# EricBAndrews/Fast-Needleman-Wunsch

Measured on AMD Instinct MI355X. Metric: GCUPS (DP cell updates/s) on NxN NW fill, bit-exact score, higher is better.
Workload: dtype int32; 1 GPU; nw_fill_262144x262144; n1=262144, n2=262144, table_bytes=274880004100, layout=row-major int32, pitch 262208, waves=auto, parallelism=single GPU, kernel=panels

## Files before the change

fast-needleman-wunsch_amd/csrc/nw_sw.hip:

```cpp
#include <hip/hip_runtime.h>
#include <stdint.h>

#include <algorithm>

#include "nw_internal.h"

namespace nw {

__global__ __launch_bounds__(256) void nw_sw_best(const int32_t *__restrict__ smax, int32_t nstrips,
                                                  int32_t *__restrict__ best, uint64_t *__restrict__ key) {
    __shared__ int32_t red[256];
    int32_t m = 0;
    for (int32_t p = threadIdx.x; p < nstrips; p += 256) m = max(m, smax[p]);
    red[threadIdx.x] = m;
    __syncthreads();
    for (int s = 128; s > 0; s >>= 1) {
        if ((int)threadIdx.x < s) red[threadIdx.x] = max(red[threadIdx.x], red[threadIdx.x + s]);
        __syncthreads();
    }
    if (threadIdx.x == 0) {
        best[0] = red[0];
        *key = ~0ull;
    }
}

constexpr int kLocRows = 64;
constexpr int kLocMaxGrid = 4096;
__global__ __launch_bounds__(256) void nw_sw_locate(const int32_t *__restrict__ table, int64_t pitch,
                                                    int64_t n1, int64_t n2, int64_t col0, int32_t strip_cols,
                                                    const int32_t *__restrict__ smax, int32_t nstrips,
                                                    const int32_t *__restrict__ best,
                                                    uint64_t *__restrict__ key) {
    const int32_t b = *best;
    if (b <= 0) return;
    __shared__ unsigned long long kmin;
    if (threadIdx.x == 0) kmin = ~0ull;
    __syncthreads();
    const int64_t nblk = (n2 + kLocRows) / kLocRows;
    for (int64_t y = blockIdx.x; y < nblk; y += gridDim.x) {
        const int64_t r0 = y * kLocRows;
        const int nr = (int)min((int64_t)kLocRows, n2 + 1 - r0);
        for (int32_t p = 0; p < nstrips; ++p) {
            if (smax[p] != b) continue;
            for (int32_t x = threadIdx.x; x < strip_cols; x += 256) {
                const int64_t c = col0 + (int64_t)p * strip_cols + x;
                if (c > n1) break;
                const int32_t *col = table + r0 * pitch + c;
                int first = kLocRows;
#pragma unroll 16
                for (int rr = kLocRows - 1; rr >= 0; --rr) {
                    const int32_t v = rr < nr ? col[rr * pitch] : 0;
                    first = v == b ? rr : first;
                }
                if (first < kLocRows)
                    atomicMin(&kmin, ((unsigned long long)(r0 + first) << 32) | (unsigned long long)c);
            }
        }
    }
    __syncthreads();
    if (threadIdx.x == 0 && kmin != ~0ull) atomicMin((unsigned long long *)key, kmin);
}

int launch_sw_locate(const int32_t *table, int64_t pitch, int64_t n1, int64_t n2, int64_t col0,
                     int32_t strip_cols, const int32_t *smax, int32_t nstrips, uint64_t *key, int32_t *best,
                     void *stream) {
    hipStream_t s = (hipStream_t)stream;
    hipLaunchKernelGGL(nw_sw_best, dim3(1), dim3(256), 0, s, smax, nstrips, best, key);
    const int64_t grid = std::min<int64_t>((n2 + kLocRows) / kLocRows, kLocMaxGrid);
    hipLaunchKernelGGL(nw_sw_locate, dim3((unsigned)grid), dim3(256), 0, s, table, pitch, n1, n2, col0, strip_cols,
                       smax, nstrips, best, key);
    return (int)hipGetLastError();
}

__global__ __launch_bounds__(64) void nw_sw_fixup(int32_t *__restrict__ t, int64_t pitch,
                                                  const uint8_t *__restrict__ s1, const uint8_t *__restrict__ s2,
                                                  int32_t match, int32_t mismatch, int32_t gap, int64_t i0,
                                                  int64_t i1, int64_t j0, int64_t j1, int64_t col0, int32_t width,
                                                  int32_t *__restrict__ smax) {
    if (threadIdx.x != 0) return;
    for (int64_t i = i0; i <= i1; ++i) {
        int32_t left = t[i * pitch + j0 - 1];
        for (int64_t j = j0; j <= j1; ++j) {
            const int32_t d = t[(i - 1) * pitch + j - 1], u = t[(i - 1) * pitch + j];
            const int32_t sc = s1[j - 1] == s2[i - 1] ? match : mismatch;
            const int32_t v = max(max(0, d + sc), max(u + gap, left + gap));
            t[i * pitch + j] = v;
            left = v;
            atomicMax(smax + (j - col0) / width, v);
        }
    }
}

int64_t sw_half_corner(int32_t match, int32_t mismatch, int64_t n1, int64_t n2, int64_t *k) {
    const int64_t m = std::max(match, mismatch);
    if (m <= 0) {
        *k = INT64_MAX;
        return 0;
    }
    *k = (65536 + m - 1) / m;
    return std::max<int64_t>(0, n2 - *k + 1) * std::max<int64_t>(0, n1 - *k + 1);
}

int launch_sw_fixup(int32_t *table, int64_t pitch, int64_t n1, int64_t n2, const uint8_t *s1, const uint8_t *s2,
                    int32_t match, int32_t mismatch, int32_t gap, int64_t col0, int32_t strip_cols, int32_t *smax,
                    void *stream) {
    int64_t k = 0;
    if (sw_half_corner(match, mismatch, n1, n2, &k) == 0) return (int)hipSuccess;
    hipLaunchKernelGGL(nw_sw_fixup, dim3(1), dim3(64), 0, (hipStream_t)stream, table, pitch, s1, s2, match,
                       mismatch, gap, k, n2, k, n1, col0, strip_cols, smax);
    return (int)hipGetLastError();
}

constexpr int kTbR = 64;
constexpr int kTbBMax = 256;
constexpr int kTbWMax = 2 * kTbBMax + 1;
constexpr int kTbThreads = 512;
constexpr int kChain = 32;
enum : uint8_t { kCStop = 0, kCDiag = 1, kCUp = 2, kCLeft = 3, kCBad = 4 };
enum : uint32_t { kXCont = 0, kXStop = 1, kXOut = 2, kXBad = 3 };
__device__ __forceinline__ uint32_t xrec(uint32_t kind, uint32_t cnt, uint32_t r, uint32_t x) {
    return kind | (cnt << 2) | (r << 12) | (x << 19);
}

enum : int { kTbLocal = 0, kTbGlobal = 1, kTbBlock = 2 };

__host__ __device__ __forceinline__ int64_t tb_shift(int64_t k, int64_t is, int64_t js, int32_t B, int32_t aim,
                                                     int64_t row0 = 0) {
    if (!aim) return 0;
    const int64_t gi = is + row0;
    const int64_t num = js - gi, lim = B / 2;
    const int64_t mag = num < 0 ? -num : num;
    if (kTbR * mag > lim * gi) return (num < 0 ? -k : k) * lim;
    return k * kTbR * num / gi;
}

template <typename F>
__device__ __forceinline__ uint32_t tb_walk(const uint8_t *cd, int W, int x, F &&emit) {
    int r = kTbR - 1;
    uint32_t cnt = 0;
    for (;;) {
        const uint8_t c = cd[r * W + x];
        if (c == kCStop) return xrec(kXStop, cnt, r, x);
        if (c == kCBad) return xrec(kXBad, cnt, r, x);
        const int nx = c == kCUp ? x + 1 : c == kCLeft ? x - 1 : x;
        if (nx < 0 || nx >= W) return xrec(kXOut, cnt, r, x);
        emit(c == kCDiag ? 0u : c == kCUp ? 1u : 2u);
        ++cnt;
        if (c != kCLeft && r == 0) return xrec(kXCont, cnt, 0, nx);
        r = c == kCLeft ? r : r - 1;
        x = nx;
    }
}

template <int KIND>
__global__ __launch_bounds__(kTbThreads) void nw_tb_windows(const int32_t *__restrict__ table, int64_t pitch,
                                                            int64_t n1, const uint8_t *__restrict__ s1,
                                                            const uint8_t *__restrict__ s2, int32_t match,
                                                            int32_t mismatch, int32_t gap, int64_t is, int64_t js,
                                                            int32_t B, int32_t aim, int64_t row0,
                                                            uint8_t *__restrict__ codes,
                                                            uint32_t *__restrict__ exits) {
    __shared__ uint8_t cd[kTbR * kTbWMax];
    const int W = 2 * B + 1;
    const int k = blockIdx.x;
    const int64_t i0 = is - (int64_t)(k + 1) * kTbR + 1;
    const int64_t dj = js - is + i0 - B - tb_shift(k, is, js, B, aim, row0);
    const int ncell = kTbR * W;
    uint8_t *gcd = codes + (int64_t)k * ncell;
#pragma unroll 4
    for (int e = threadIdx.x; e < ncell; e += kTbThreads) {
        const int r = e / W, x = e - r * W;
        const int64_t i = i0 + r, j = dj + r + x;
        const bool in = i >= 1 && j >= 1 && j <= n1;
        const int64_t ic = in ? i : 1, jc = in ? j : 1;
        const int32_t *row = table + ic * pitch;
        const int32_t t = row[jc], td = row[jc - 1 - pitch], tu = row[jc - pitch], tl = row[jc - 1];
        const int32_t sc = s1[jc - 1] == s2[ic - 1] ? match : mismatch;
        const uint8_t mv = t == td + sc ? kCDiag : t == tu + gap ? kCUp : t == tl + gap ? kCLeft : kCBad;
        uint8_t c;
        if (KIND == kTbLocal) {
            c = in && t > 0 ? mv : kCStop;
        } else if (KIND == kTbBlock) {
            c = in ? mv
                   : i == 0 && j >= 0 && j <= n1 ? kCStop
                   : j == 0 && i > 0 ? kCUp
                                     : kCBad;
        } else {
            c = in ? mv
                   : i == 0 && j == 0 ? kCStop
                   : i == 0 && j > 0 && j <= n1 ? kCLeft
                   : j == 0 && i > 0 ? kCUp
                                     : kCBad;
        }
        cd[e] = c;
        gcd[e] = c;
    }
    __syncthreads();
    for (int x = threadIdx.x; x < W; x += kTbThreads) exits[(int64_t)k * W + x] = tb_walk(cd, W, x, [](uint32_t) {});
}

__global__ __launch_bounds__(1024) void nw_tb_chain(const uint32_t *__restrict__ exits, int32_t nwin, int32_t B,
                                                    int32_t aim, int64_t is, int64_t js, int64_t row0,
                                                    int64_t ops_cap, int64_t *__restrict__ wentry,
                                                    int64_t *__restrict__ ctl) {
    __shared__ uint32_t ex[kChain * kTbWMax];
    __shared__ int64_t st[3];
    const int W = 2 * B + 1;
    const int tid = threadIdx.x;
    if (tid == 0) {
        st[0] = B;
        st[1] = ctl[0];
        st[2] = 0;
    }
    for (int k0 = 0; k0 < nwin; k0 += kChain) {
        const int nk = min(kChain, nwin - k0);
        for (int e = tid; e < nk * W; e += 1024) ex[e] = exits[(int64_t)k0 * W + e];
        __syncthreads();
        if (tid == 0) {
            int x = (int)st[0];
            int64_t off = st[1];
            for (int kk = 0; kk < nk; ++kk) {
                const int k = k0 + kk;
                wentry[2 * k] = x;
                wentry[2 * k + 1] = off;
                const uint32_t rec = ex[kk * W + x];
                const uint32_t kind = rec & 3u, cnt = (rec >> 2) & 1023u, r = (rec >> 12) & 127u, xx = rec >> 19;
                off += cnt;
                const int64_t ck = tb_shift(k, is, js, B, aim, row0);
                x = (int)xx;
                if (kind == kXCont && k + 1 < nwin) {
                    x += (int)(tb_shift(k + 1, is, js, B, aim, row0) - ck);
                    if (x >= 0 && x < W) continue;
                }
                const int64_t i0 = is - (int64_t)(k + 1) * kTbR + 1, dj = js - is + i0 - B - ck;
                ctl[1] = off > ops_cap ? 4 : (int64_t)kind;
                ctl[2] = kind == kXCont ? i0 - 1 : i0 + r;
                ctl[3] = kind == kXCont ? dj - 1 + xx : dj + r + xx;
                ctl[4] = k + 1;
                ctl[0] = off;
                st[2] = 1;
                break;
            }
            st[0] = x;
            st[1] = off;
        }
        __syncthreads();
        if (st[2]) break;
    }
}

__global__ __launch_bounds__(256) void nw_tb_emit(const uint8_t *__restrict__ codes, int32_t B,
                                                  const int64_t *__restrict__ wentry, const int64_t *__restrict__ ctl,
                                                  uint8_t *__restrict__ ops) {
    __shared__ uint32_t cdw[kTbR * kTbWMax / 4 + 1];
    __shared__ uint8_t ob[2 * kTbR + kTbWMax + 8];
    __shared__ int32_t nop;
    const int k = blockIdx.x;
    if (k >= ctl[4] || ctl[1] == 4) return;
    const int W = 2 * B + 1, ncell = kTbR * W;
    const uint32_t *g = (const uint32_t *)(codes + (int64_t)k * ncell);
    for (int e = threadIdx.x; e < ncell / 4; e += 256) cdw[e] = g[e];
    __syncthreads();
    if (threadIdx.x == 0) {
        int q = 0;
        tb_walk((const uint8_t *)cdw, W, (int)wentry[2 * k], [&](uint32_t op) { ob[q++] = (uint8_t)op; });
        nop = q;
    }
    __syncthreads();
    const int64_t off = wentry[2 * k + 1];
    for (int m = threadIdx.x; m < nop; m += 256) ops[off + m] = ob[m];
}

size_t sw_tb_scratch_bytes(int32_t maxwin, int32_t band) {
    const size_t W = 2 * (size_t)band + 1;
    return 64 + (size_t)maxwin * (16 + 4 * W + kTbR * W);
}

static int32_t tb_steep_cap(int64_t is, int64_t js, int32_t B, int64_t row0) {
    const int64_t gi = is + row0;
    const int64_t num = js - gi, mag = num < 0 ? -num : num, lim = B / 2;
    const int64_t drift = (kTbR * mag - lim * gi) / gi;
    return drift <= 0 ? INT32_MAX : (int32_t)std::min<int64_t>(B / drift + 2, INT32_MAX);
}

template <int KIND>
static int run_traceback(const int32_t *table, int64_t pitch, int64_t n1, const uint8_t *s1, const uint8_t *s2,
                         int32_t match, int32_t mismatch, int32_t gap, int64_t end_i, int64_t end_j, uint8_t *ops,
                         int64_t ops_cap, void *scratch, int32_t maxwin, int32_t band, int32_t aim, int64_t *info,
                         void *stream, int64_t row0 = 0) {
    hipStream_t s = (hipStream_t)stream;
    for (int q = 0; q < 10; ++q) info[q] = 0;
    if (band < 1 || band > kTbBMax || maxwin < 1) return (int)hipErrorInvalidValue;
    const int W = 2 * band + 1;
    int64_t *ctl = (int64_t *)scratch;
    int64_t *wentry = ctl + 8;
    uint32_t *exits = (uint32_t *)(wentry + 2 * (size_t)maxwin);
    uint8_t *codes = (uint8_t *)(exits + (size_t)maxwin * W);
    hipError_t e = hipMemsetAsync(ctl, 0, 64, s);
    if (e != hipSuccess) return (int)e;
    int64_t ci = end_i, cj = end_j, h[8] = {0, 0, 0, 0, 0, 0, 0, 0};
    for (;;) {
        if (ci <= 0 || cj <= 0) {
            info[1] = ci;
            info[2] = cj;
            break;
        }
        int32_t nwin = (int32_t)std::min<int64_t>((ci + kTbR) / kTbR, maxwin);
        if (aim) nwin = std::min(nwin, tb_steep_cap(ci, cj, band, row0));
        hipLaunchKernelGGL(nw_tb_windows<KIND>, dim3((unsigned)nwin), dim3(kTbThreads), 0, s, table, pitch, n1, s1,
                           s2, match, mismatch, gap, ci, cj, band, aim, row0, codes, exits);
        hipLaunchKernelGGL(nw_tb_chain, dim3(1), dim3(1024), 0, s, exits, nwin, band, aim, ci, cj, row0, ops_cap,
                           wentry, ctl);
        hipLaunchKernelGGL(nw_tb_emit, dim3((unsigned)nwin), dim3(256), 0, s, codes, band, wentry, ctl, ops);
        if ((e = hipGetLastError()) != hipSuccess) return (int)e;
        if ((e = hipMemcpyAsync(h, ctl, sizeof h, hipMemcpyDeviceToHost, s)) != hipSuccess) return (int)e;
        if ((e = hipStreamSynchronize(s)) != hipSuccess) return (int)e;
        info[4] += 1;
        info[5] += nwin;
        info[0] = h[0];
        if (h[1] == kXStop) {
            info[1] = h[2];
            info[2] = h[3];
            break;
        }
        if (h[1] == kXBad || h[1] == 4) {
            info[3] = h[1] == 4 ? 1 : 2;
            info[1] = h[2];
            info[2] = h[3];
            break;
        }
        ci = h[2];
        cj = h[3];
    }
    if ((KIND == kTbGlobal || (KIND == kTbBlock && info[1] > 0)) && info[3] == 0 && (info[1] > 0 || info[2] > 0)) {
        const int64_t tail = info[1] > 0 ? info[1] : info[2];
        if (info[1] < 0 || info[2] < 0 || (info[1] > 0 && info[2] > 0)) {
            info[3] = 2;
        } else if (info[0] + tail > ops_cap) {
            info[3] = 1;
        } else {
            if ((e = hipMemsetAsync(ops + info[0], info[1] > 0 ? 1 : 2, (size_t)tail, s)) != hipSuccess)
                return (int)e;
            info[0] += tail;
            info[6] = tail;
            info[1] = info[2] = 0;
        }
    }
    return (int)hipSuccess;
}

int run_sw_traceback(const int32_t *table, int64_t pitch, int64_t n1, const uint8_t *s1, const uint8_t *s2,
                     int32_t match, int32_t mismatch, int32_t gap, int64_t end_i, int64_t end_j, uint8_t *ops,
                     int64_t ops_cap, void *scratch, int32_t maxwin, int32_t band, int64_t *info, void *stream) {
    return run_traceback<kTbLocal>(table, pitch, n1, s1, s2, match, mismatch, gap, end_i, end_j, ops, ops_cap, scratch,
                                   maxwin, band, 0, info, stream);
}

int run_nw_traceback(const int32_t *table, int64_t pitch, int64_t n1, int64_t n2, const uint8_t *s1,
                     const uint8_t *s2, int32_t match, int32_t mismatch, int32_t gap, uint8_t *ops, int64_t ops_cap,
                     void *scratch, int32_t maxwin, int32_t band, int32_t aim, int64_t *info, void *stream) {
    return run_traceback<kTbGlobal>(table, pitch, n1, s1, s2, match, mismatch, gap, n2, n1, ops, ops_cap, scratch,
                                    maxwin, band, aim, info, stream);
}

int run_nw_traceback_block(const int32_t *table, int64_t pitch, int64_t n1, int64_t rows, int64_t row0,
                           const uint8_t *s1, const uint8_t *s2, int32_t match, int32_t mismatch, int32_t gap,
                           uint8_t *ops, int64_t ops_cap, void *scratch, int32_t maxwin, int32_t band, int32_t aim,
                           int64_t *info, void *stream) {
    return run_traceback<kTbBlock>(table, pitch, n1, s1, s2, match, mismatch, gap, rows, n1, ops, ops_cap, scratch,
                                   maxwin, band, aim, info, stream, row0);
}

int64_t tb_shift_host(int64_t k, int64_t is, int64_t js, int32_t B, int32_t aim, int64_t row0) {
    return tb_shift(k, is, js, B, aim, row0);
}

}
```

fast-needleman-wunsch_amd/csrc/nw_traceback.cpp:

```cpp
#include <algorithm>
#include <cstring>

#include "nw_host_int.h"

using namespace nwh;

namespace {

int tb_workspace(nw_ctx *c, size_t ops, int64_t rows, int32_t band, int32_t *maxwin) {
    int st;
    if ((st = grow((void **)&c->ops, &c->ops_cap, ops)) != NW_OK) return st;
    *maxwin = (int32_t)std::min<int64_t>(*maxwin, rows / 64 + 1);
    return grow((void **)&c->tbscratch, &c->tbscratch_cap, nw::sw_tb_scratch_bytes(*maxwin, band));
}

int tb_elapsed(nw_ctx *c, hipStream_t s, float *ms) {
    NW_HIP_TRY(hipEventRecord(c->ev1, s));
    NW_HIP_TRY(hipStreamSynchronize(s));
    NW_HIP_TRY(hipEventElapsedTime(ms, c->ev0, c->ev1));
    return NW_OK;
}

void set_alignment(nw_alignment *out, int64_t end_i, int64_t end_j, const int64_t *info, float ms, int status) {
    out->end_i = end_i;
    out->end_j = end_j;
    out->n_ops = info[0];
    out->begin_i = info[1];
    out->begin_j = info[2];
    out->traceback_ms = ms;
    out->status = status;
}

}

extern "C" {

int nw_sw_traceback(nw_ctx *c, const int8_t *d_s1, int64_t n1, const int8_t *d_s2, int64_t n2,
                    const nw_params *p, const int32_t *d_t, int64_t pitch, int64_t end_i, int64_t end_j,
                    uint8_t *host_ops, int64_t ops_cap, nw_alignment *out) {
    if (!c || !d_t || !p || !out || n1 < 0 || n2 < 0 || end_i < 0 || end_j < 0 || end_i > n2 || end_j > n1)
        return NW_ERR_ARG;
    if ((end_j > 0 && !d_s1) || (end_i > 0 && !d_s2) || (ops_cap > 0 && !host_ops) || ops_cap < 0)
        return NW_ERR_ARG;
    if (!valid_params(p) || p->mode != NW_MODE_SW) return NW_ERR_ARG;
    NW_HIP_TRY(hipSetDevice(c->device));
    NW_HIP_TRY(hipDeviceSynchronize());
    const int32_t band = std::max(1, std::min(256, env_int("NW_TB_BAND", nw::kTbBandDefault)));
    int32_t maxwin = std::max(1, env_int("NW_TB_MAXWIN", nw::kTbMaxWinDefault));
    int st;
    const size_t need = (size_t)std::max<int64_t>(end_i + end_j + 1, 1);
    if ((st = tb_workspace(c, need, end_i, band, &maxwin)) != NW_OK) return st;
    NW_HIP_TRY(hipEventRecord(c->ev0, nullptr));
    int64_t info[10];
    const int he = nw::run_sw_traceback(d_t, pitch, n1, (const uint8_t *)d_s1, (const uint8_t *)d_s2, p->match,
                                        p->mismatch, p->gap, end_i, end_j, c->ops, (int64_t)need, c->tbscratch,
                                        maxwin, band, info, nullptr);
    if (he != hipSuccess) {
        std::fprintf(stderr, "libnwhip: SW traceback failed: %s\n", hipGetErrorString((hipError_t)he));
        return NW_ERR_HIP;
    }
    float ms = 0.f;
    if ((st = tb_elapsed(c, nullptr, &ms)) != NW_OK) return st;
    if (env_set("NW_TB_DEBUG"))
        std::fprintf(stderr, "nw_sw_traceback: %lld moves, %lld rounds, %lld windows (band %d)\n", (long long)info[0],
                     (long long)info[4], (long long)info[5], band);
    std::memset(out, 0, sizeof *out);
    set_alignment(out, end_i, end_j, info, ms, info[3] == 0 ? NW_OK : NW_ERR_HIP);
    NW_HIP_TRY(hipMemcpy(&out->score, d_t + end_i * pitch + end_j, 4, hipMemcpyDeviceToHost));
    if (info[3] != 0) return out->status;
    if (info[0] > ops_cap) return NW_ERR_ARG;
    if (info[0] > 0) {
        NW_HIP_TRY(hipMemcpy(host_ops, c->ops, (size_t)info[0], hipMemcpyDeviceToHost));
        std::reverse(host_ops, host_ops + info[0]);
    }
    return NW_OK;
}

int nw_traceback(nw_ctx *c, const int8_t *d_s1, int64_t n1, const int8_t *d_s2, int64_t n2, const nw_params *p,
                 const int32_t *d_t, int64_t pitch, const nw_tb_opts *o, void *stream, uint8_t *host_ops,
                 int64_t ops_cap, nw_alignment *out, nw_tb_stats *stats) {
    int32_t band = 0, maxwin = 0, aim = 0;
    int st = tb_args(n1, n2, p, o, host_ops, ops_cap, out, &band, &maxwin, &aim);
    if (st != NW_OK) return st;
    if (!c || !d_t || pitch < n1 + 1 || (n1 > 0 && !d_s1) || (n2 > 0 && !d_s2)) return NW_ERR_ARG;
    hipStream_t s = (hipStream_t)stream;
    NW_HIP_TRY(hipSetDevice(c->device));
    if ((st = tb_workspace(c, (size_t)std::max<int64_t>(n1 + n2, 1), n2, band, &maxwin)) != NW_OK) return st;
    NW_HIP_TRY(hipEventRecord(c->ev0, s));
    int64_t info[10];
    const int he = nw::run_nw_traceback(d_t, pitch, n1, n2, (const uint8_t *)d_s1, (const uint8_t *)d_s2, p->match,
                                        p->mismatch, p->gap, c->ops, n1 + n2, c->tbscratch, maxwin, band, aim, info,
                                        stream);
    if (he != hipSuccess) {
        std::fprintf(stderr, "libnwhip: traceback failed: %s\n", hipGetErrorString((hipError_t)he));
        return NW_ERR_HIP;
    }
    std::memset(out, 0, sizeof *out);
    out->end_i = n2;
    out->end_j = n1;
    if (stats) {
        stats->rounds = (int32_t)info[4];
        stats->windows = (int32_t)info[5];
        stats->band = band;
        stats->max_windows = maxwin;
        stats->tail_ops = info[6];
    }
    const bool ok = info[3] == 0;
    NW_HIP_TRY(hipMemcpyAsync(&out->score, d_t + n2 * pitch + n1, 4, hipMemcpyDeviceToHost, s));
    if (ok && info[0] > 0) NW_HIP_TRY(hipMemcpyAsync(host_ops, c->ops, (size_t)info[0], hipMemcpyDeviceToHost, s));
    float ms = 0.f;
    if ((st = tb_elapsed(c, s, &ms)) != NW_OK) return st;
    if (!ok) {
        out->traceback_ms = ms;
        out->status = NW_ERR_TABLE;
        return NW_ERR_TABLE;
    }
    set_alignment(out, n2, n1, info, ms, NW_OK);
    std::reverse(host_ops, host_ops + info[0]);
    return NW_OK;
}

int nw_traceback_block(nw_ctx *c, const int8_t *d_s1, int64_t n1, const int8_t *d_s2_block, int64_t rows,
                       int64_t row0, const nw_params *p, const int32_t *d_t, int64_t pitch, const nw_tb_opts *o,
                       void *stream, uint8_t *host_ops, int64_t ops_cap, nw_alignment *out, nw_tb_stats *stats) {
    int32_t band = 0, maxwin = 0, aim = 0;
    int st = tb_args(n1, rows, p, o, host_ops, ops_cap, out, &band, &maxwin, &aim);
    if (st != NW_OK) return st;
    if (row0 < 0 || row0 + rows >= INT32_MAX) return NW_ERR_ARG;
    if (!c || !d_t || pitch < n1 + 1 || (n1 > 0 && !d_s1) || (rows > 0 && !d_s2_block)) return NW_ERR_ARG;
    if (row0 == 0) {
        st = nw_traceback(c, d_s1, n1, d_s2_block, rows, p, d_t, pitch, o, stream, host_ops, ops_cap, out, stats);
        return st;
    }
    hipStream_t s = (hipStream_t)stream;
    NW_HIP_TRY(hipSetDevice(c->device));
    if ((st = tb_workspace(c, (size_t)std::max<int64_t>(n1 + rows, 1), rows, band, &maxwin)) != NW_OK) return st;
    NW_HIP_TRY(hipEventRecord(c->ev0, s));
    int64_t info[10];
    const int he = nw::run_nw_traceback_block(d_t, pitch, n1, rows, row0, (const uint8_t *)d_s1,
                                              (const uint8_t *)d_s2_block, p->match, p->mismatch, p->gap, c->ops,
                                              n1 + rows, c->tbscratch, maxwin, band, aim, info, stream);
    if (he != hipSuccess) {
        std::fprintf(stderr, "libnwhip: traceback failed: %s\n", hipGetErrorString((hipError_t)he));
        return NW_ERR_HIP;
    }
    std::memset(out, 0, sizeof *out);
    if (stats) {
        stats->rounds = (int32_t)info[4];
        stats->windows = (int32_t)info[5];
        stats->band = band;
        stats->max_windows = maxwin;
        stats->tail_ops = info[6];
    }
    const bool ok = info[3] == 0;
    NW_HIP_TRY(hipMemcpyAsync(&out->score, d_t + rows * pitch + n1, 4, hipMemcpyDeviceToHost, s));
    if (ok && info[0] > 0) NW_HIP_TRY(hipMemcpyAsync(host_ops, c->ops, (size_t)info[0], hipMemcpyDeviceToHost, s));
    float ms = 0.f;
    if ((st = tb_elapsed(c, s, &ms)) != NW_OK) return st;
    if (!ok) {
        out->end_i = row0 + rows;
        out->end_j = n1;
        out->traceback_ms = ms;
        out->status = NW_ERR_TABLE;
        return NW_ERR_TABLE;
    }
    set_alignment(out, row0 + rows, n1, info, ms, NW_OK);
    out->begin_i = row0 + info[1];
    std::reverse(host_ops, host_ops + info[0]);
    return NW_OK;
}

int64_t nw_debug_tb_shift(int64_t k, int64_t is, int64_t js, int32_t band, int32_t aim, int64_t row0) {
    return nw::tb_shift_host(k, is, js, band, aim, row0);
}

}
```

Baseline: 1522 GCUPS.

## Batch traceback rounds on device and stage window table reads through LDS rows

Traceback now keeps its loop state on the device: a begin kernel seeds the control block, and the window and chain kernels read their position from it and exit early once finished. The host enqueues growing batches of rounds between synchronisations instead of one sync per round. The window kernel loads table rows into a shared-memory ring with prefetch instead of doing four scattered global loads per cell, and the score is returned through the control block. None of this touches the fill kernel that the GCUPS metric measures, and speculative batches launch idle kernels.

```diff
diff --git a/fast-needleman-wunsch_amd/csrc/nw_sw.hip b/fast-needleman-wunsch_amd/csrc/nw_sw.hip
--- a/fast-needleman-wunsch_amd/csrc/nw_sw.hip
+++ b/fast-needleman-wunsch_amd/csrc/nw_sw.hip
@@ -2,6 +2,7 @@
 #include <stdint.h>
 
 #include <algorithm>
+#include <cstdlib>
 
 #include "nw_internal.h"
 
@@ -114,7 +115,7 @@
 constexpr int kTbR = 64;
 constexpr int kTbBMax = 256;
 constexpr int kTbWMax = 2 * kTbBMax + 1;
-constexpr int kTbThreads = 512;
+constexpr int kTbThreads = 576;
 constexpr int kChain = 32;
 enum : uint8_t { kCStop = 0, kCDiag = 1, kCUp = 2, kCLeft = 3, kCBad = 4 };
 enum : uint32_t { kXCont = 0, kXStop = 1, kXOut = 2, kXBad = 3 };
@@ -137,80 +138,188 @@
 template <typename F>
 __device__ __forceinline__ uint32_t tb_walk(const uint8_t *cd, int W, int x, F &&emit) {
     int r = kTbR - 1;
+    int at = r * W + x;
     uint32_t cnt = 0;
     for (;;) {
-        const uint8_t c = cd[r * W + x];
+        const uint32_t c = cd[at];
         if (c == kCStop) return xrec(kXStop, cnt, r, x);
         if (c == kCBad) return xrec(kXBad, cnt, r, x);
-        const int nx = c == kCUp ? x + 1 : c == kCLeft ? x - 1 : x;
-        if (nx < 0 || nx >= W) return xrec(kXOut, cnt, r, x);
-        emit(c == kCDiag ? 0u : c == kCUp ? 1u : 2u);
+        const int dx = (c == kCUp) - (c == kCLeft), nx = x + dx;
+        if ((unsigned)nx >= (unsigned)W) return xrec(kXOut, cnt, r, x);
+        emit(c - kCDiag);
         ++cnt;
-        if (c != kCLeft && r == 0) return xrec(kXCont, cnt, 0, nx);
-        r = c == kCLeft ? r : r - 1;
+        if (c != kCLeft) {
+            if (r == 0) return xrec(kXCont, cnt, 0, nx);
+            --r;
+            at -= W;
+        }
+        at += dx;
         x = nx;
     }
 }
+static_assert(kCDiag == 1 && kCUp == 2 && kCLeft == 3, "tb_walk emits code - 1");
+
+__host__ __device__ __forceinline__ bool tb_running(int64_t state) { return state == kXCont || state == kXOut; }
+
+__host__ __device__ __forceinline__ int32_t tb_steep_cap(int64_t is, int64_t js, int32_t B, int64_t row0) {
+    const int64_t gi = is + row0;
+    const int64_t num = js - gi, mag = num < 0 ? -num : num, lim = B / 2;
+    const int64_t drift = (kTbR * mag - lim * gi) / gi;
+    if (drift <= 0) return INT32_MAX;
+    const int64_t cap = B / drift + 2;
+    return cap < INT32_MAX ? (int32_t)cap : INT32_MAX;
+}
+
+__host__ __device__ __forceinline__ int32_t tb_nwin(int64_t is, int64_t js, int32_t B, int32_t aim, int64_t row0,
+                                                    int32_t maxwin) {
+    int64_t n = (is + kTbR) / kTbR;
+    n = n < maxwin ? n : maxwin;
+    if (aim) {
+        const int32_t cap = tb_steep_cap(is, js, B, row0);
+        n = n < cap ? n : cap;
+    }
+    return (int32_t)n;
+}
+
+__global__ void nw_tb_begin(const int32_t *__restrict__ table, int64_t pitch, int64_t ci, int64_t cj,
+                            int64_t *__restrict__ ctl) {
+    if (threadIdx.x != 0) return;
+    ctl[0] = 0;
+    ctl[1] = ci <= 0 || cj <= 0 ? kXStop : kXCont;
+    ctl[2] = ci;
+    ctl[3] = cj;
+    ctl[4] = ctl[5] = ctl[6] = 0;
+    ctl[7] = table[ci * pitch + cj];
+}
+
+constexpr int kTbCh = 8;
+constexpr int kTbRingW = kTbWMax + 3;
+constexpr int kTbLd = (kTbWMax + 2 + 63) / 64;
+constexpr int kTbAhead = 2;
+static_assert(kTbR % kTbCh == 0 && (kTbR * kTbWMax) % 4 == 0 && kTbThreads >= 64 * kTbCh && kTbThreads >= kTbWMax,
+              "window chunks");
 
 template <int KIND>
 __global__ __launch_bounds__(kTbThreads) void nw_tb_windows(const int32_t *__restrict__ table, int64_t pitch,
                                                             int64_t n1, const uint8_t *__restrict__ s1,
                                                             const uint8_t *__restrict__ s2, int32_t match,
-                                                            int32_t mismatch, int32_t gap, int64_t is, int64_t js,
-                                                            int32_t B, int32_t aim, int64_t row0,
+                                                            int32_t mismatch, int32_t gap, int32_t B, int32_t aim,
+                                                            int64_t row0, int32_t maxwin,
+                                                            const int64_t *__restrict__ ctl,
                                                             uint8_t *__restrict__ codes,
                                                             uint32_t *__restrict__ exits) {
-    __shared__ uint8_t cd[kTbR * kTbWMax];
+    __shared__ uint32_t cdw[kTbR * kTbWMax / 4];
+    __shared__ int32_t ring[(kTbCh + 1) * kTbRingW];
+    __shared__ uint8_t s1c[kTbR + kTbWMax];
+    if (!tb_running(ctl[1])) return;
+    const int64_t is = ctl[2], js = ctl[3];
+    const int k = blockIdx.x;
+    if (k >= tb_nwin(is, js, B, aim, row0, maxwin)) return;
+    uint8_t *cd = (uint8_t *)cdw;
     const int W = 2 * B + 1;
-    const int k = blockIdx.x;
     const int64_t i0 = is - (int64_t)(k + 1) * kTbR + 1;
     const int64_t dj = js - is + i0 - B - tb_shift(k, is, js, B, aim, row0);
     const int ncell = kTbR * W;
-    uint8_t *gcd = codes + (int64_t)k * ncell;
-#pragma unroll 4
-    for (int e = threadIdx.x; e < ncell; e += kTbThreads) {
-        const int r = e / W, x = e - r * W;
-        const int64_t i = i0 + r, j = dj + r + x;
-        const bool in = i >= 1 && j >= 1 && j <= n1;
-        const int64_t ic = in ? i : 1, jc = in ? j : 1;
-        const int32_t *row = table + ic * pitch;
-        const int32_t t = row[jc], td = row[jc - 1 - pitch], tu = row[jc - pitch], tl = row[jc - 1];
-        const int32_t sc = s1[jc - 1] == s2[ic - 1] ? match : mismatch;
-        const uint8_t mv = t == td + sc ? kCDiag : t == tu + gap ? kCUp : t == tl + gap ? kCLeft : kCBad;
-        uint8_t c;
-        if (KIND == kTbLocal) {
-            c = in && t > 0 ? mv : kCStop;
-        } else if (KIND == kTbBlock) {
-            c = in ? mv
-                   : i == 0 && j >= 0 && j <= n1 ? kCStop
-                   : j == 0 && i > 0 ? kCUp
-                                     : kCBad;
-        } else {
-            c = in ? mv
-                   : i == 0 && j == 0 ? kCStop
-                   : i == 0 && j > 0 && j <= n1 ? kCLeft
-                   : j == 0 && i > 0 ? kCUp
-                                     : kCBad;
-        }
-        cd[e] = c;
-        gcd[e] = c;
-    }
-    __syncthreads();
+    const int lane = threadIdx.x & 63, wv = threadIdx.x >> 6;
+    for (int q = threadIdx.x; q < kTbR + W - 1; q += kTbThreads) {
+        const int64_t j = dj + q;
+        s1c[q] = j >= 1 && j <= n1 ? s1[j - 1] : 0;
+    }
+    auto load_row = [&](int r, int32_t(&v)[kTbLd]) {
+        const int64_t i = i0 + r, jb = dj + r - 1;
+        const int32_t *rp = table + (i >= 0 ? i : 0) * pitch;
+#pragma unroll
+        for (int m = 0; m < kTbLd; ++m) {
+            const int xs = lane + 64 * m;
+            const int64_t j = jb + xs;
+            v[m] = xs < W + 2 && i >= 0 && j >= 0 && j <= n1 ? rp[j] : 0;
+        }
+    };
+    auto put_row = [&](int r, const int32_t(&v)[kTbLd]) {
+        int32_t *d = ring + ((r + 1) % (kTbCh + 1)) * kTbRingW;
+#pragma unroll
+        for (int m = 0; m < kTbLd; ++m) {
+            const int xs = lane + 64 * m;
+            if (xs < W + 2) d[xs] = v[m];
+        }
+    };
+    int32_t v[kTbAhead][kTbLd];
+    if (wv == kTbCh - 1) {
+        load_row(-1, v[0]);
+        put_row(-1, v[0]);
+    }
+    const bool rows = wv < kTbCh;
+#pragma unroll
+    for (int ch = 0; ch < kTbAhead; ++ch)
+        if (rows) load_row(ch * kTbCh + wv, v[ch]);
+#pragma unroll
+    for (int ch = 0; ch < kTbR / kTbCh; ++ch) {
+        const int r = ch * kTbCh + wv;
+        if (rows) {
+            put_row(r, v[ch % kTbAhead]);
+            if (ch + kTbAhead < kTbR / kTbCh) load_row(r + kTbAhead * kTbCh, v[ch % kTbAhead]);
+        }
+        __syncthreads();
+        const int64_t i = i0 + r;
+        const int32_t *cur = ring + ((r + 1) % (kTbCh + 1)) * kTbRingW + 1;
+        const int32_t *abv = ring + (r % (kTbCh + 1)) * kTbRingW + 1;
+        const uint8_t c2 = rows && i >= 1 ? s2[i - 1] : 0;
+#pragma unroll
+        for (int m = 0; m < kTbLd; ++m) {
+            const int x = lane + 64 * m;
+            if (!rows || x >= W) continue;
+            const int64_t j = dj + r + x;
+            const bool in = i >= 1 && j >= 1 && j <= n1;
+            const int32_t t = cur[x], td = abv[x], tu = abv[x + 1], tl = cur[x - 1];
+            const int32_t sc = s1c[r + x] == c2 ? match : mismatch;
+            const uint8_t mv = t == td + sc ? kCDiag : t == tu + gap ? kCUp : t == tl + gap ? kCLeft : kCBad;
+            uint8_t c;
+            if (KIND == kTbLocal) {
+                c = in && t > 0 ? mv : kCStop;
+            } else if (KIND == kTbBlock) {
+                c = in ? mv
+                       : i == 0 && j >= 0 && j <= n1 ? kCStop
+                       : j == 0 && i > 0 ? kCUp
+                                         : kCBad;
+            } else {
+                c = in ? mv
+                       : i == 0 && j == 0 ? kCStop
+                       : i == 0 && j > 0 && j <= n1 ? kCLeft
+                       : j == 0 && i > 0 ? kCUp
+                                         : kCBad;
+            }
+            cd[r * W + x] = c;
+        }
+        __syncthreads();
+    }
+    uint32_t *gcd = (uint32_t *)(codes + (int64_t)k * ncell);
+    for (int e = threadIdx.x; e < ncell / 4; e += kTbThreads) gcd[e] = cdw[e];
     for (int x = threadIdx.x; x < W; x += kTbThreads) exits[(int64_t)k * W + x] = tb_walk(cd, W, x, [](uint32_t) {});
 }
 
-__global__ __launch_bounds__(1024) void nw_tb_chain(const uint32_t *__restrict__ exits, int32_t nwin, int32_t B,
-                                                    int32_t aim, int64_t is, int64_t js, int64_t row0,
-                                                    int64_t ops_cap, int64_t *__restrict__ wentry,
-                                                    int64_t *__restrict__ ctl) {
+__global__ __launch_bounds__(1024) void nw_tb_chain(const uint32_t *__restrict__ exits, int32_t B, int32_t aim,
+                                                    int64_t row0, int32_t maxwin, int64_t ops_cap,
+                                                    int64_t *__restrict__ wentry, int64_t *__restrict__ ctl) {
     __shared__ uint32_t ex[kChain * kTbWMax];
-    __shared__ int64_t st[3];
+    __shared__ int64_t st[6];
     const int W = 2 * B + 1;
     const int tid = threadIdx.x;
     if (tid == 0) {
         st[0] = B;
         st[1] = ctl[0];
         st[2] = 0;
+        st[3] = tb_running(ctl[1]);
+        st[4] = ctl[2];
+        st[5] = ctl[3];
+        if (!st[3]) ctl[4] = 0;
+    }
+    __syncthreads();
+    if (!st[3]) return;
+    const int64_t is = st[4], js = st[5];
+    const int32_t nwin = tb_nwin(is, js, B, aim, row0, maxwin);
+    if (tid == 0) {
+        ctl[5] += 1;
+        ctl[6] += nwin;
     }
     for (int k0 = 0; k0 < nwin; k0 += kChain) {
         const int nk = min(kChain, nwin - k0);
@@ -233,9 +342,13 @@
                     if (x >= 0 && x < W) continue;
                 }
                 const int64_t i0 = is - (int64_t)(k + 1) * kTbR + 1, dj = js - is + i0 - B - ck;
-                ctl[1] = off > ops_cap ? 4 : (int64_t)kind;
-                ctl[2] = kind == kXCont ? i0 - 1 : i0 + r;
-                ctl[3] = kind == kXCont ? dj - 1 + xx : dj + r + xx;
+                const int64_t ni = kind == kXCont ? i0 - 1 : i0 + r;
+                const int64_t nj = kind == kXCont ? dj - 1 + xx : dj + r + xx;
+                ctl[1] = off > ops_cap                                ? 4
+                         : tb_running(kind) && (ni <= 0 || nj <= 0) ? (int64_t)kXStop
+                                                                    : (int64_t)kind;
+                ctl[2] = ni;
+                ctl[3] = nj;
                 ctl[4] = k + 1;
                 ctl[0] = off;
                 st[2] = 1;
@@ -276,11 +389,12 @@
     return 64 + (size_t)maxwin * (16 + 4 * W + kTbR * W);
 }
 
-static int32_t tb_steep_cap(int64_t is, int64_t js, int32_t B, int64_t row0) {
-    const int64_t gi = is + row0;
-    const int64_t num = js - gi, mag = num < 0 ? -num : num, lim = B / 2;
-    const int64_t drift = (kTbR * mag - lim * gi) / gi;
-    return drift <= 0 ? INT32_MAX : (int32_t)std::min<int64_t>(B / drift + 2, INT32_MAX);
+constexpr int kTbBatch = 6;
+constexpr int kTbBatchMax = 64;
+static int tb_env(const char *name, int dflt) {
+    const char *e = std::getenv(name);
+    const int v = e && *e ? std::atoi(e) : 0;
+    return v >= 1 ? v : dflt;
 }
 
 template <int KIND>
@@ -296,42 +410,42 @@
     int64_t *wentry = ctl + 8;
     uint32_t *exits = (uint32_t *)(wentry + 2 * (size_t)maxwin);
     uint8_t *codes = (uint8_t *)(exits + (size_t)maxwin * W);
-    hipError_t e = hipMemsetAsync(ctl, 0, 64, s);
-    if (e != hipSuccess) return (int)e;
-    int64_t ci = end_i, cj = end_j, h[8] = {0, 0, 0, 0, 0, 0, 0, 0};
-    for (;;) {
-        if (ci <= 0 || cj <= 0) {
-            info[1] = ci;
-            info[2] = cj;
-            break;
-        }
-        int32_t nwin = (int32_t)std::min<int64_t>((ci + kTbR) / kTbR, maxwin);
-        if (aim) nwin = std::min(nwin, tb_steep_cap(ci, cj, band, row0));
-        hipLaunchKernelGGL(nw_tb_windows<KIND>, dim3((unsigned)nwin), dim3(kTbThreads), 0, s, table, pitch, n1, s1,
-                           s2, match, mismatch, gap, ci, cj, band, aim, row0, codes, exits);
-        hipLaunchKernelGGL(nw_tb_chain, dim3(1), dim3(1024), 0, s, exits, nwin, band, aim, ci, cj, row0, ops_cap,
-                           wentry, ctl);
-        hipLaunchKernelGGL(nw_tb_emit, dim3((unsigned)nwin), dim3(256), 0, s, codes, band, wentry, ctl, ops);
+    hipError_t e;
+    hipLaunchKernelGGL(nw_tb_begin, dim3(1), dim3(64), 0, s, table, pitch, end_i, end_j, ctl);
+    const int64_t max_rounds = end_i + end_j + 2;
+    int batch = tb_env("NW_TB_BATCH", kTbBatch);
+    const int batch_max = std::max(batch, tb_env("NW_TB_BATCH_MAX", kTbBatchMax));
+    int64_t h[8] = {0, end_i <= 0 || end_j <= 0 ? (int64_t)kXStop : (int64_t)kXCont, end_i, end_j, 0, 0, 0, 0};
+    bool fetched = false;
+    while (tb_running(h[1])) {
+        if (h[5] >= max_rounds) return (int)hipErrorUnknown;
+        const unsigned grid = (unsigned)tb_nwin(h[2], h[3], band, 0, row0, maxwin);
+        for (int q = 0; q < batch; ++q) {
+            hipLaunchKernelGGL(nw_tb_windows<KIND>, dim3(grid), dim3(kTbThreads), 0, s, table, pitch, n1, s1, s2,
+                               match, mismatch, gap, band, aim, row0, maxwin, ctl, codes, exits);
+            hipLaunchKernelGGL(nw_tb_chain, dim3(1), dim3(1024), 0, s, exits, band, aim, row0, maxwin, ops_cap,
+                               wentry, ctl);
+            hipLaunchKernelGGL(nw_tb_emit, dim3(grid), dim3(256), 0, s, codes, band, wentry, ctl, ops);
+        }
         if ((e = hipGetLastError()) != hipSuccess) return (int)e;
         if ((e = hipMemcpyAsync(h, ctl, sizeof h, hipMemcpyDeviceToHost, s)) != hipSuccess) return (int)e;
         if ((e = hipStreamSynchronize(s)) != hipSuccess) return (int)e;
-        info[4] += 1;
-        info[5] += nwin;
-        info[0] = h[0];
-        if (h[1] == kXStop) {
-            info[1] = h[2];
-            info[2] = h[3];
-            break;
-        }
-        if (h[1] == kXBad || h[1] == 4) {
-            info[3] = h[1] == 4 ? 1 : 2;
-            info[1] = h[2];
-            info[2] = h[3];
-            break;
-        }
-        ci = h[2];
-        cj = h[3];
-    }
+        fetched = true;
+        batch = std::min(2 * batch, batch_max);
+    }
+    if (!fetched) {
+        if ((e = hipGetLastError()) != hipSuccess) return (int)e;
+        if ((e = hipMemcpyAsync(h, ctl, sizeof h, hipMemcpyDeviceToHost, s)) != hipSuccess) return (int)e;
+        if ((e = hipStreamSynchronize(s)) != hipSuccess) return (int)e;
+    }
+    info[0] = h[0];
+    info[1] = h[2];
+    info[2] = h[3];
+    info[4] = h[5];
+    info[5] = h[6];
+    info[7] = h[7];
+    if (h[1] == kXBad || h[1] == 4) info[3] = h[1] == 4 ? 1 : 2;
+    else if (h[1] != kXStop) return (int)hipErrorUnknown;
     if ((KIND == kTbGlobal || (KIND == kTbBlock && info[1] > 0)) && info[3] == 0 && (info[1] > 0 || info[2] > 0)) {
         const int64_t tail = info[1] > 0 ? info[1] : info[2];
         if (info[1] < 0 || info[2] < 0 || (info[1] > 0 && info[2] > 0)) {
diff --git a/fast-needleman-wunsch_amd/csrc/nw_traceback.cpp b/fast-needleman-wunsch_amd/csrc/nw_traceback.cpp
--- a/fast-needleman-wunsch_amd/csrc/nw_traceback.cpp
+++ b/fast-needleman-wunsch_amd/csrc/nw_traceback.cpp
@@ -59,20 +59,21 @@
         std::fprintf(stderr, "libnwhip: SW traceback failed: %s\n", hipGetErrorString((hipError_t)he));
         return NW_ERR_HIP;
     }
+    const bool give = info[3] == 0 && info[0] > 0 && info[0] <= ops_cap;
+    NW_HIP_TRY(hipEventRecord(c->ev1, nullptr));
+    if (give) NW_HIP_TRY(hipMemcpyAsync(host_ops, c->ops, (size_t)info[0], hipMemcpyDeviceToHost, nullptr));
+    NW_HIP_TRY(hipStreamSynchronize(nullptr));
     float ms = 0.f;
-    if ((st = tb_elapsed(c, nullptr, &ms)) != NW_OK) return st;
+    NW_HIP_TRY(hipEventElapsedTime(&ms, c->ev0, c->ev1));
     if (env_set("NW_TB_DEBUG"))
         std::fprintf(stderr, "nw_sw_traceback: %lld moves, %lld rounds, %lld windows (band %d)\n", (long long)info[0],
                      (long long)info[4], (long long)info[5], band);
     std::memset(out, 0, sizeof *out);
     set_alignment(out, end_i, end_j, info, ms, info[3] == 0 ? NW_OK : NW_ERR_HIP);
-    NW_HIP_TRY(hipMemcpy(&out->score, d_t + end_i * pitch + end_j, 4, hipMemcpyDeviceToHost));
+    out->score = (int32_t)info[7];
     if (info[3] != 0) return out->status;
     if (info[0] > ops_cap) return NW_ERR_ARG;
-    if (info[0] > 0) {
-        NW_HIP_TRY(hipMemcpy(host_ops, c->ops, (size_t)info[0], hipMemcpyDeviceToHost));
-        std::reverse(host_ops, host_ops + info[0]);
-    }
+    if (give) std::reverse(host_ops, host_ops + info[0]);
     return NW_OK;
 }
 
@@ -106,7 +107,7 @@
         stats->tail_ops = info[6];
     }
     const bool ok = info[3] == 0;
-    NW_HIP_TRY(hipMemcpyAsync(&out->score, d_t + n2 * pitch + n1, 4, hipMemcpyDeviceToHost, s));
+    out->score = (int32_t)info[7];
     if (ok && info[0] > 0) NW_HIP_TRY(hipMemcpyAsync(host_ops, c->ops, (size_t)info[0], hipMemcpyDeviceToHost, s));
     float ms = 0.f;
     if ((st = tb_elapsed(c, s, &ms)) != NW_OK) return st;
@@ -153,7 +154,7 @@
         stats->tail_ops = info[6];
     }
     const bool ok = info[3] == 0;
-    NW_HIP_TRY(hipMemcpyAsync(&out->score, d_t + rows * pitch + n1, 4, hipMemcpyDeviceToHost, s));
+    out->score = (int32_t)info[7];
     if (ok && info[0] > 0) NW_HIP_TRY(hipMemcpyAsync(host_ops, c->ops, (size_t)info[0], hipMemcpyDeviceToHost, s));
     float ms = 0.f;
     if ((st = tb_elapsed(c, s, &ms)) != NW_OK) return st;
```

Result: no change. 1526 GCUPS, median of 3 (+0.3%).
